# relife957/FastApriori

Measured on AMD Instinct MI355X. Metric: itemsets/sec (mining wall-clock), T10I4D100M min_sup=0.001, higher is better.
Workload: dtype int32/uint64-bitmap (exact integer counts); 1 GPU; model=T10I4D100M, global_batch=100000000, parallelism=dp1, n_itemsets=33139, min_count=100000

## Files before the change

### csrc/hip/fa_hip.h

```cpp
#pragma once
#include <hip/hip_runtime.h>
#include <stdint.h>

#define FA_API extern "C" __attribute__((visibility("default")))

#define FA_LAUNCH_RET() return (int)hipGetLastError()

namespace fa {

constexpr int kWave = 64;

__device__ __forceinline__ int lane_id() { return (int)(threadIdx.x & 63); }

__device__ __forceinline__ uint32_t popc64_acc(uint64_t x, uint32_t acc) {
  return acc + (uint32_t)__popc((uint32_t)x) + (uint32_t)__popc((uint32_t)(x >> 32));
}

__device__ __forceinline__ int wave_scan_incl_dpp(int v) {
  const int lane = (int)(threadIdx.x & 63);
  const int r = lane & 15;
  int t;
  t = __builtin_amdgcn_update_dpp(0, v, 0x111, 0xf, 0xf, false); if (r >= 1) v += t;
  t = __builtin_amdgcn_update_dpp(0, v, 0x112, 0xf, 0xf, false); if (r >= 2) v += t;
  t = __builtin_amdgcn_update_dpp(0, v, 0x114, 0xf, 0xf, false); if (r >= 4) v += t;
// ... 157 lines not shown
  for (int i = 0, j = 0; i < k - 1; ++i, ++j) {
    if (j == p) ++j;
    const int32_t x = a[i], y = s[j];
    if (x != y) return x < y ? -1 : 1;
  }
  return 0;
}

struct DlDesc;

}

FA_API int fa_hip_dl_plan(const fa::DlDesc* desc, int L, long long* ctl, int F1, int32_t* item_map, void* rec,
                          int64_t max_pieces, int32_t* part, int64_t part_cap, int32_t* gpre, int64_t gpre_cap,
                          int sw, hipStream_t st);
FA_API int fa_hip_count_slab_rec_cls(const int64_t* roff, const int32_t* ranks, const int32_t* src, int64_t ncols,
                                     const int32_t* item_map, int F1, int n_used, const int32_t* gpre,
                                     const void* rec, int G, int C, const int32_t* wword, uint32_t* out, int sw,
                                     int n_wg, const uint64_t* bm, int64_t Wp, hipStream_t st,
                                     const int32_t* bm_rows, const int32_t* g_dev, int cls);
```

### csrc/hip/gen.hip

```cpp
#include <hipcub/hipcub.hpp>

#include <algorithm>
#include <cmath>

#include "fa_hip.h"
#include "../host/fa_dl.h"
#include "../host/fa_limits.h"
#include "../host/fa_slab.h"

namespace fa {

__device__ __forceinline__ uint64_t ag_mix(uint64_t x) {
  x ^= x >> 33; x *= 0xff51afd7ed558ccdull; x ^= x >> 33; x *= 0xc4ceb9fe1a85ec53ull; x ^= x >> 33;
  return x;
}

__device__ __forceinline__ uint64_t ag_hash_drop(const int32_t* __restrict__ r, int m, int skip) {
  uint64_t h = 0x9E3779B97F4A7C15ull ^ (uint64_t)(m - 1);
  for (int q = 0; q < m; ++q)
    if (q != skip) h = ag_mix(h ^ (uint32_t)r[q]);
  return h;
}

__device__ __forceinline__ bool ag_eq_drop(const int32_t* __restrict__ a, const int32_t* __restrict__ b, int m,
// ... 845 lines not shown
  int64_t Cl[kDlMaxL], C = 0, R = 0;
  for (int l = 0; l < *L; ++l) { Cl[l] = desc[l].C; C += desc[l].C; R += desc[l].n; }
  const int64_t n_used = ch[kDlNUsed];
  const int Lp = *Lp_out = slab_tail_cut(Cl, *L, n_used, lds, accb_rule);
  if (Lp == *L) return false;
  const bool ends = ch[kDlEmpty] || (g_tail_levels > 0 && *L == g_tail_levels);
  if (ends && C <= P->rec_cap && C <= P->out_cap && 8 * ((R + 255) / 256) <= P->part_cap &&
      slab_pack_width(n_used, C, lds, accb_pack, cap, pad) == 16 && C <= *cap) {
    *sw = 16;
    return true;
  }
  dl_tail_cut(desc, L, Lp, ch);
  return false;
}

static void dl_post(DlPost* P, const DlDesc* desc, int L, long long* ctl, long long* ch, int F1,
                    double accb_rule, double accb_pack, double lds, hipStream_t st) {
  P->done = 0;
  if (ch[kDlStop] && ch[kDlLevels] == 0) return;
  if (ch[kDlOverBound] || ch[kDlMulti] || ch[kDlEnd] || L < 1) return;
  int64_t cap = 0;
  int sw = 0, pad = 0, Lp = L;
  const bool packed = accb_pack > 0.0 && dl_tail(P, desc, &L, ch, accb_rule, accb_pack, lds, &Lp, &sw, &cap, &pad);
  int64_t C = 0, R = 0;
  for (int l = 0; l < L; ++l) { C += desc[l].C; R += desc[l].n; }
  const int64_t n_used = ch[kDlNUsed];
  P->C = C;
  if (C < 1 || C > P->rec_cap || C > P->out_cap || 8 * ((R + 255) / 256) > P->part_cap) return;
  double accb = accb_rule;
  if (packed) {
    accb = accb_pack;
  } else {
    sw = slab_width(n_used, C, P->lds_budget, accb_rule, &cap);
    if (sw == 0 || C > cap) return;
    if (!P->wword) slab_acc_upgrade(n_used, C, P->lds_budget, P->accb, &sw, &cap, &accb);
  }
  P->accb = accb;
  if (fa_hip_dl_plan(desc, L, ctl, F1, P->item_map, P->rec, C, P->part, P->part_cap, P->gpre, P->gpre_cap,
                     slab_layout(sw, pad), st) != 0) {
    if (packed) dl_tail_cut(desc, &L, Lp, ch);
    return;
  }
  (void)hipMemsetAsync(P->out, 0, 4 * (size_t)C, st);
  P->sw = slab_layout(sw, pad);
  P->cap = cap;
  P->done = 1;
  P->trim = 0;
  if (!P->trim_ok || P->T <= 0) {
  } else if (!P->len_hist || P->T < P->trim_min_rows) {
    if (!P->len_hist && P->T >= P->trim_min_rows) return;
  } else {
    const uint64_t* mk = reinterpret_cast<const uint64_t*>(ch + kDlBits);
    double num = 0.0, den = 0.0;
    for (int r = 0; r < F1; ++r) {
      if (P->alive[r]) den += (double)P->c1[r];
      if ((mk[r >> 6] >> (r & 63)) & 1ull) num += (double)P->c1[r];
    }
    if (den > 0.0) {
      double est_rows = 0.0, est_nnz = 0.0;
      trim_estimate(P->len_hist, kTrimHist, num / den, (int)P->k, &est_rows, &est_nnz);
      const double T = (double)std::max<int64_t>(P->T, 1), nnz = (double)std::max<int64_t>(P->nnz, 1);
      P->trim = (est_rows < P->trim_rows_frac * T || est_nnz < P->trim_nnz_frac * nnz) ? 1 : 0;
    }
  }
  if (P->trim) return;
  const int64_t W = (P->ncols + 63) / 64, nslabs = (W + sw - 1) / sw;
  const bool weighted = P->wword != nullptr;
  const int64_t nacc = slab_acc_count(C, slab_acc_bytes(P->accb, weighted));
  P->n_wg = slab_workgroups(nslabs, (int64_t)P->lds_kernel,
                            slab_kernel_lds_pack(n_used, sw, pad, slab_acc_words(nacc), slab_map_lds(F1)));
  if (fa_hip_count_slab_rec_cls(P->roff, P->ranks, P->src, P->ncols, P->item_map, F1, (int)n_used, P->gpre, P->rec,
                                0, (int)C, P->wword, P->out, slab_layout(sw, pad), (int)P->n_wg, nullptr, 0, st,
                                nullptr,
                                reinterpret_cast<const int32_t*>(ctl + kDlPiecesI32),
                                slab_acc_mode(P->accb, weighted)) != 0)
    return;
  P->done = 2;
}

FA_API int fa_hip_dl_more(int F1, void* ws, int64_t ws_bytes, int64_t ws_used, long long* ctl, long long* ctl_host,
                          double growth, int max_levels, double lds, double accb, int64_t n1_bound, fa::DlDesc* desc,
                          int64_t* info, hipStream_t st, void* post) {
  using namespace fa;
  auto al = [](int64_t b) { return (b + 255) & ~(int64_t)255; };
  const int nw = (F1 + 63) / 64;
  char* const w0 = static_cast<char*>(ws);
  char* w = w0 + ws_used;
  const int LM = std::min(max_levels, kDlMaxLevels);
  const int64_t acc_max = (int64_t)(lds / accb);
  const DlPost* const tp = static_cast<const DlPost*>(post);
  const double accb_pack = tp && !tp->wword && F1 <= kSlabMapMaxF1 ? g_tail_accb : 0.0;
  int64_t nb = n1_bound;
// ... 87 lines not shown
  desc[0].C = ctl_host[kDlCl];
  desc[0].base = 0;
  const int L = (int)ctl_host[kDlLevels];
  for (int l = 1; l < L; ++l) {
    DlDesc& d = desc[l];
    d.P = desc[l - 1].rows;
    d.cnt = (int64_t)(intptr_t)lv[l].cnt;
    d.off = (int64_t)(intptr_t)lv[l].off;
    d.rows = (int64_t)(intptr_t)lv[l].rows;
    d.m = lv[l].m;
    d.n = ctl_host[kDlNl + l];
    d.C = ctl_host[kDlCl + l];
    d.base = desc[l - 1].base + desc[l - 1].C;
  }
  info[0] = w - w0;
  if (post) dl_post(static_cast<DlPost*>(post), desc, L, ctl, ctl_host, F1, accb, accb_pack, lds, st);
  FA_LAUNCH_RET();
}
```

### fastapriori_amd/models/apriori.py

```python
from __future__ import annotations

import gc
import math
import os
import time
from dataclasses import dataclass

import numpy as np
import torch

from .. import ops
from ..ops.host import apriori_gen
from ..parallel.comm import Comm
from ..tuning import TUNING
from ..utils.jvm import item_tiebreak_key, min_count
from ..utils.metrics import Logger, Timer, roctx_range
from .data import MiningResult, TransactionShard

HORIZONTAL_PAIRS_PER_S = 2.0e11
GRAM_WORDPAIRS_PER_S = 1.7e13
F1_SKETCH_MIN_VOCAB = 1 << 20
F1_HIST_READBACK = 1 << 16
_TRIU_CACHE: dict = {}
_POW10 = 10 ** np.arange(1, 11, dtype=np.int64)
# ... 269 lines not shown
        S = Pm.device_level_state(self._dev)
        F1 = self._F1
        lds = Pm.dl_lds_budget(F1)
        unit = db["wword"] is None
        self._dl_mp_accb = 2.0 if TUNING.dl_acc16 and unit else 4.0
        acc8 = int(TUNING.dl_acc8_bundles) if unit else 0
        if int(self._count_view(db)["ncols"]) < TUNING.dl_acc8_min_rows:
            acc8 = 0
        accb = self._dl_accb = 1.0 if acc8 == 1 else 2.0 if TUNING.dl_acc16_bundles and unit else 4.0
        self._dl_cnt_accb = 1.0 if acc8 == 2 else accb
        counters = 1 if self.cand_par else max(1, self.comm.world_size)
        tail_rows = int(self.stats["n_lines"]) // counters
        self._dl_tail_accb = 0.0
        if TUNING.dl_tail_bundle and unit and Pm.slab_map_lds(F1) > 0 and tail_rows >= TUNING.dl_acc8_min_rows:
            self._dl_tail_accb = 1.0 if int(TUNING.dl_acc8_bundles) else 2.0 if TUNING.dl_acc16_bundles else 4.0
        c_bound = int(lds // accb)
        st = torch.cuda.current_stream(self._dev).cuda_stream
        f2 = self._f2_dev
        m0, k = 2, 3
        if f2 is None:
            last = np.ascontiguousarray(levels[-1], dtype=np.int32)
            m0, k = last.shape[1], last.shape[1] + 1
            f2 = self._resume_rows = torch.from_numpy(last.reshape(-1, m0)).to(self._dev)
        if self._f2_n_dev is not None:
            P0, n_src, n_const, n_bound = f2.data_ptr(), self._f2_n_dev.data_ptr(), 0, self._f2_bound
        else:
            P0, n_src, n_const, n_bound = f2.data_ptr(), None, int(f2.shape[0]), int(f2.shape[0])
        if self.ckpt is not None and self._ckpt_deferred:
            self._result_items(result)
            n_host = next((i for i, lv in enumerate(levels) if lv is None), len(levels))
# ... 15 lines not shown
                tail_levels = 0
                if self.cfg.max_level and self.cfg.max_level - k + 1 <= max_lv:
                    max_lv = tail_levels = self.cfg.max_level - k + 1
                if not TUNING.bundle_levels or k - 1 > TUNING.bundle_max_prefix:
                    max_lv = 1
                post = TUNING.dl_post and max_lv > 1
                S.rows_hint = int(self._count_view(db)["ncols"])
                if post:
                    self._dl_post_setup(S, db, k, F1, c_bound, n_bound, lds)
                if pend:
                    self._dl_stage(S, pend)
                with roctx_range("gen"):
                    c = Pm.dl_bundle_gen(S, P0, n_src, n_const, n_bound, m0, F1, c_bound, lds, TUNING.bundle_growth,
                                         max_lv, st, post=post, accb=accb,
                                         tail_accb=self._dl_tail_accb if post else 0.0,
                                         tail_levels=tail_levels if max_lv > 1 else 0)
                if c[K.kDlOverBound]:
                    raise RuntimeError(f"device bundle at level {k}: |F_{k - 1}| exceeds its bound {n_bound}")
                if c[K.kDlEnd]:
                    break
                multi = None
                if c[K.kDlMulti]:
                    multi = self._dl_multipass(S, db, k, F1, c, P0, n_src, n_const, n_bound, m0, lds, st)
                    if multi is None:
                        nxt = k
                        break
                    c = multi[0]
                L, n_used = int(c[K.kDlLevels]), int(c[K.kDlNUsed])
                Cs = S.desc["C"][:L].copy()
                C = int(Cs.sum())
                done = int(S.post.done) if post else 0
# ... 985 lines not shown
```

### fastapriori_amd/ops/_native.py

```python
from __future__ import annotations

import ctypes as C
import os
import threading

from . import build as _build

_lock = threading.Lock()
_host = None
_hip = None

i32, i64, u64, dbl = C.c_int32, C.c_int64, C.c_uint64, C.c_double
vp, cp = C.c_void_p, C.c_char_p
I64P = C.POINTER(C.c_int64)
IP = C.POINTER(C.c_int)

_HOST_SIGS = {
    "fa_parse_file": (vp, [cp, i64, i64, C.c_int, C.c_int, IP]),
    "fa_parse_buffer": (vp, [cp, i64, C.c_int, C.c_int]),
    "fa_file_size": (i64, [cp]),
    "fa_next_line_start": (i64, [cp, i64, i64]),
    "fa_chunk_scan": (None, [vp, i64, vp]),
    "fa_txndb_info": (None, [vp, vp]),
    "fa_txndb_export": (None, [vp, vp, vp, vp, C.c_int]),
    "fa_txndb_export_dict": (None, [vp, vp, vp, vp, C.c_int]),
    "fa_hash_tokens": (None, [vp, vp, i64, vp, C.c_int]),
    "fa_txndb_free": (None, [vp]),
    "fa_hash_bytes": (u64, [cp, i64]),
    "fa_quest_generate": (vp, [i64, i64, dbl, dbl, i64, i64, u64, C.c_int, C.c_int]),
    "fa_zipf_generate": (vp, [i64, i64, dbl, dbl, i64, dbl, dbl, i64, u64, C.c_int]),
    "fa_zipf_write": (C.c_int, [cp, i64, dbl, dbl, i64, dbl, dbl, i64, u64, C.c_int, C.c_int]),
    "fa_quest_write": (C.c_int, [cp, i64, dbl, dbl, i64, i64, u64, C.c_int, C.c_int]),
    "fa_apriori_gen": (vp, [vp, i64, C.c_int, C.c_int, vp]),
    "fa_cands_export": (None, [vp, vp, vp, vp]),
    "fa_cands_free": (None, [vp]),
    "fa_level_plan": (C.c_int, [vp, vp, i64, vp, vp, i32, vp, vp, i64, vp, i64, vp]),
    "fa_slab_width": (C.c_int, [i64, i64, dbl, dbl, I64P]),
    "fa_slab_total_limit": (i64, [i64, dbl, dbl]),
    "fa_slab_map_lds": (i64, [i64]),
    "fa_slab_workgroups": (i64, [i64, i64, C.c_int, i64, C.c_int, i64, i64]),
    "fa_slab_acc_mode": (C.c_int, [dbl, C.c_int, i64, I64P]),
    "fa_slab_acc_upgrade": (C.c_int, [i64, i64, dbl, dbl, C.POINTER(C.c_int), I64P, C.POINTER(dbl)]),
    "fa_slab_row_off": (i64, [C.c_int, C.c_int, i64]),
    "fa_slab_row_col": (C.c_int, [C.c_int, C.c_int, i64]),
    "fa_slab_rows_bytes": (i64, [C.c_int, C.c_int, i64]),
    "fa_slab_layout": (C.c_int, [C.c_int, C.c_int]),
    "fa_slab_pack_width": (C.c_int, [i64, i64, dbl, dbl, I64P, C.POINTER(C.c_int)]),
    "fa_slab_tail_cut": (C.c_int, [vp, C.c_int, i64, dbl, dbl]),
    "fa_trim_estimate": (None, [vp, i64, dbl, C.c_int, C.POINTER(dbl), C.POINTER(dbl)]),
    "fa_dl_layout": (cp, [C.c_int, I64P]),
    "fa_limits": (cp, [C.c_int, I64P]),
# ... 56 lines not shown
    "fa_hip_lr_rows": (C.c_int, [vp, vp, vp, i64, vp, C.c_int, vp, i64, vp]),
    "fa_hip_compress_regs_bc": (C.c_int, [vp, vp, vp, vp, i64, vp, vp, vp, vp, vp, i64, C.c_int, vp]),
    "fa_hip_block_counts_rows": (C.c_int, [vp, vp, vp, i64, vp, i64, C.c_int, vp, vp]),
    "fa_hip_block_bsum": (C.c_int, [vp, i64, i64, C.c_int, vp, vp]),
    "fa_hip_compress_staged": (C.c_int, [vp, vp, vp, i64, vp, vp, vp, vp, vp]),
    "fa_hip_compress_staged64": (C.c_int, [vp, vp, vp, i64, vp, vp, vp, vp, C.c_int, vp]),
    "fa_hip_count_slab_rec_cls": (C.c_int, [vp, vp, vp, i64, vp, C.c_int, C.c_int, vp, vp, C.c_int, C.c_int, vp,
                                            vp, C.c_int, C.c_int, vp, i64, vp, vp, vp, C.c_int]),
    "fa_hip_dl_level0": (C.c_int, [vp, vp, i64, i64, C.c_int, C.c_int, vp, i64, vp, vp, i64, dbl, dbl, vp, C.c_int,
                                   vp]),
    "fa_hip_dl_more": (C.c_int, [C.c_int, vp, i64, i64, vp, vp, dbl, C.c_int, dbl, dbl, i64, vp, vp, vp, vp]),
    "fa_hip_dl_plan": (C.c_int, [vp, C.c_int, vp, C.c_int, vp, vp, i64, vp, i64, vp, i64, C.c_int, vp]),
    "fa_hip_set_lane_deal": (None, [C.c_int]),
    "fa_hip_set_dl_tail": (None, [dbl, C.c_int]),
    "fa_hip_set_piece_part": (C.c_int, [C.c_int, C.c_int]),
    "fa_hip_dl_gpre_need": (i64, [vp, C.c_int]),
    "fa_hip_dl_plan_window": (C.c_int, [vp, C.c_int, vp, C.c_int, vp, vp, i64, vp, i64, vp, i64, i64, i64, C.c_int,
                                        vp]),
    "fa_hip_dl_plan_window_bits": (C.c_int, [vp, C.c_int, vp, C.c_int, vp, vp, vp, i64, vp, i64, vp, i64, i64, i64,
                                             C.c_int, vp]),
    "fa_hip_dl_chunk_bits": (C.c_int, [vp, C.c_int, C.c_int, vp, vp]),
    "fa_hip_dl_threshold": (C.c_int, [vp, C.c_int, vp, i64, vp, vp, vp, vp, vp, vp, i64, vp]),
    "fa_hip_trim_scan_count": (C.c_int, [vp, vp, i64, vp, C.c_int, C.c_int, vp, vp, vp, vp, vp]),
    "fa_hip_trim_emit": (C.c_int, [vp, vp, vp, C.c_int, i64, vp, vp, vp, vp, vp, vp, vp, vp]),
    "fa_hip_compress_wave": (C.c_int, [vp, vp, vp, vp, i64, vp, vp, vp, C.c_int, vp, vp]),
    "fa_hip_compress_lds": (C.c_int, [vp, vp, vp, vp, i64, vp, vp, vp, vp, vp, vp]),
    "fa_hip_dedup_probe": (C.c_int, [vp, vp, vp, i64, vp, vp, vp]),
    "fa_hip_row_hash": (C.c_int, [vp, vp, i64, vp, vp, vp]),
    "fa_hip_build_bitmaps": (C.c_int, [vp, vp, vp, i64, i32, i64, C.c_int, C.c_int, vp, vp, vp, C.c_int, vp]),
    "fa_hip_block_counts": (C.c_int, [vp, vp, i64, i32, vp, vp, C.c_int, vp]),
# ... 97 lines not shown
```

### fastapriori_amd/ops/build.py

```python
from __future__ import annotations

import glob
import hashlib
import os
import shutil
import subprocess
import sys

HERE = os.path.dirname(os.path.abspath(__file__))
ROOT = os.path.dirname(os.path.dirname(HERE))
CSRC = os.path.join(ROOT, "csrc")
HOST_LIB = os.path.join(HERE, "libfa_host.so")
HIP_LIB = os.path.join(HERE, "libfa_hip.so")
ARCH = os.environ.get("PYTORCH_ROCM_ARCH", "gfx950").split(";")[0] or "gfx950"

HOST_FLAGS = ["-O3", "-std=c++17", "-shared", "-fPIC", "-pthread", "-mpopcnt", "-fvisibility=hidden", "-Wall",
              "-Wno-unused-function"]
ASAN_FLAGS = ["-O1", "-g", "-std=c++17", "-shared", "-fPIC", "-pthread", "-mpopcnt",
              "-fsanitize=address,undefined", "-fno-omit-frame-pointer"]
HIP_FLAGS = [f"--offload-arch={ARCH}", "-O3", "-std=c++17", "-shared", "-fPIC", "-fvisibility=hidden",
             "-Wno-unused-result"]
_MARKER = b"FA_BUILD_ID:"


# ... 10 lines not shown
        raise RuntimeError(f"build failed: {' '.join(cmd)}\n{r.stdout}\n{r.stderr}")


def host_sources() -> list[str]:
    return sorted(glob.glob(os.path.join(CSRC, "host", "*.cpp")))


def hip_sources() -> list[str]:
    return sorted(glob.glob(os.path.join(CSRC, "hip", "*.hip")))


def _deps(kind: str) -> list[str]:
    if kind == "host":
        return host_sources() + sorted(glob.glob(os.path.join(CSRC, "host", "*.h")))
    return hip_sources() + sorted(glob.glob(os.path.join(CSRC, "hip", "*.h"))) + [
        os.path.join(CSRC, "host", h) for h in ("fa_dl.h", "fa_limits.h", "fa_query.h", "fa_rule_measures.h",
                                                "fa_slab.h")]


def source_id(kind: str, flags: list[str] | None = None) -> str:
    if flags is None:
        flags = HOST_FLAGS if kind == "host" else HIP_FLAGS
    h = hashlib.sha256()
    for p in _deps(kind):
        h.update(os.path.relpath(p, ROOT).encode() + b"\0")
        with open(p, "rb") as f:
            h.update(f.read())
        h.update(b"\0")
    h.update(" ".join(flags).encode())
    return h.hexdigest()[:16]


# ... 43 lines not shown
```

### fastapriori_amd/ops/host.py

```python
from __future__ import annotations

import ctypes as C
from dataclasses import dataclass, field

import numpy as np

from ..config import RULE_SORTS
from ..utils.env import num_threads
from . import _native


def apriori_gen(prev: np.ndarray):
    prev = np.ascontiguousarray(prev, dtype=np.int32)
    n, m = prev.shape
    sizes = np.zeros(2, dtype=np.int64)
    lib = _native.host()
    h = lib.fa_apriori_gen(prev.ctypes.data, n, m, num_threads(), sizes.ctypes.data)
    G, Cn = int(sizes[0]), int(sizes[1])
    prefix = np.zeros(max(G, 1), dtype=np.int32)
    ext_off = np.zeros(G + 1, dtype=np.int64)
    ext = np.zeros(max(Cn, 1), dtype=np.int32)
    lib.fa_cands_export(h, prefix.ctypes.data, ext_off.ctypes.data, ext.ctypes.data)
    lib.fa_cands_free(h)
    return prefix[:G], ext_off, ext[:Cn]


@dataclass
class RuleTable:
    ante_off: np.ndarray
    ante: np.ndarray
    cons: np.ndarray
    conf: np.ndarray
    level_stats: list
    level_ms: list = field(default_factory=list)

    @property
    def n_rules(self) -> int:
        return int(self.cons.size)

# ... 141 lines not shown
```

### fastapriori_amd/ops/primitives.py

```python
from __future__ import annotations

import ctypes as C
import ctypes
import functools
import os
import time
from dataclasses import dataclass

import numpy as np
import torch

from ..tuning import TUNING
from ..utils.env import num_threads
from . import _native
from .host import rule_measures_plan, rules_gap_level, rules_not_closed

_I32, _I64 = torch.int32, torch.int64
PAIR_CHUNK_ROWS = 1 << 18


def _p(t: torch.Tensor | None) -> int | None:
    return None if t is None else t.data_ptr()


# ... 1683 lines not shown
def device_level_state(dev) -> DeviceLevelState:
    st = _DL_STATE.get(dev)
    if st is None:
        st = _DL_STATE[dev] = DeviceLevelState(dev)
    return st


def dl_lds_budget(F1: int) -> int:
    return TUNING.slab_lds_bytes - slab_map_lds(F1)




def dl_bundle_gen(S: DeviceLevelState, P0: int, n_src: int | None, n_const: int, n_bound: int, m0: int, F1: int,
                  c_bound: int, lds: int, growth: float, max_levels: int, stream: int, post: bool = False,
                  accb: float = 4.0, tail_accb: float = 0.0, tail_levels: int = 0) -> np.ndarray:
    lib, K = _native.hip(), dl()
    info = np.zeros(2, dtype=np.int64)
    for _ in range(6):
        S.desc[:] = 0
        rc = lib.fa_hip_dl_level0(P0, n_src, n_const, n_bound, m0, F1, _p(S.ws), S.ws.numel(), _p(S.ctl),
                                  _p(S.ctl_h), c_bound, float(lds), float(accb), S.info.ctypes.data,
                                  int(max_levels <= 1), stream)
        if rc == 5:
            S.grow(int(S.info[0]))
            continue
        _native.check(rc, "fa_hip_dl_level0")
        d0 = S.desc[0]
        d0["P"], d0["cnt"], d0["off"], d0["rows"], d0["m"] = P0, S.info[1], S.info[2], S.info[3], m0
        if max_levels <= 1:
            c = S.ctl_h.numpy()
            d0["n"], d0["C"], d0["base"] = c[K.kDlNl], c[K.kDlCl], 0
            return c.copy()
        S.post.done = 0
        lane_deal(lib, S.rows_hint)
        lib.fa_hip_set_dl_tail(float(tail_accb) if post else 0.0, int(tail_levels))
        rc = lib.fa_hip_dl_more(F1, _p(S.ws), S.ws.numel(), int(S.info[0]), _p(S.ctl), _p(S.ctl_h), float(growth),
                                int(max_levels), float(lds), float(accb), int(c_bound), S.desc.ctypes.data,
                                info.ctypes.data,
                                stream, ctypes.addressof(S.post) if post else None)
        if rc == 5:
            S.grow(int(info[0]))
            continue
        _native.check(rc, "fa_hip_dl_more")
        return S.ctl_h.numpy().copy()
    raise RuntimeError("device bundle generation: workspace sizing did not converge")


def set_piece_part(part: int, nparts: int) -> None:
    _native.check(_native.hip().fa_hip_set_piece_part(int(part), int(nparts)), "fa_hip_set_piece_part")


def lane_deal(lib, rows: int) -> None:
    lib.fa_hip_set_lane_deal(int(0 <= TUNING.lane_deal_min_rows <= rows))


def dl_plan(S: DeviceLevelState, L: int, F1: int, n_used: int, C: int, lds: int, dev, accb: float = 4.0,
            cnt_accb: float | None = None, pad: int = 0) -> dict:
    st = torch.cuda.current_stream(dev).cuda_stream
    sw, cap = slab_width(n_used, C, lds, accb)
    if sw == 0 or C > cap:
        raise RuntimeError(f"device bundle of {C} candidates over {n_used} items does not fit one pass")
    if cnt_accb is not None and cnt_accb < accb:
        sw_c, cap_c, accb_c = ctypes.c_int(sw), ctypes.c_int64(cap), ctypes.c_double(accb)
        _native.host().fa_slab_acc_upgrade(int(n_used), int(C), float(lds), float(cnt_accb), ctypes.byref(sw_c),
                                           ctypes.byref(cap_c), ctypes.byref(accb_c))
        sw, cap, accb = int(sw_c.value), int(cap_c.value), float(accb_c.value)
    item_map = torch.empty(max(F1, 1), dtype=_I32, device=dev)
    rec = torch.empty(12 * C + 12, dtype=_I32, device=dev)
    R = int(S.desc["n"][:L].sum())
    part = torch.empty(8 * max(1, (R + 255) // 256), dtype=_I32, device=dev)
    lib = _native.hip()
    gn = int(lib.fa_hip_dl_gpre_need(S.desc.ctypes.data, L))
    gpre = torch.empty(max(gn, 1), dtype=_I32, device=dev)
    lane_deal(lib, S.rows_hint)
    _native.check(lib.fa_hip_dl_plan(S.desc.ctypes.data, L, _p(S.ctl), F1, _p(item_map), _p(rec), C,
                                     _p(part), part.numel(), _p(gpre), gpre.numel(), slab_layout(sw, pad), st),
                  "fa_hip_dl_plan")
    out = torch.zeros(C, dtype=_I32, device=dev)
    return dict(sw=sw, pad=pad, cap=cap, item_map=item_map, rec=rec, out=out, n_used=n_used, C=C, gpre=gpre,
                accb=accb)


def dl_count_multipass(S: DeviceLevelState, F1: int, n_used: int, C: int, lds: int, roff, ranks, src, ncols: int,
                       wword, bm, bm_rows, sup_frac: float, dev, bmap=None, window_rows=None) -> torch.Tensor | None:
    acc16 = TUNING.dl_acc16 and wword is None
    accb = 2 if acc16 else 4
    sw, cap = slab_width(n_used, C, lds, accb)
    if sw == 0:
        return None
    st = _stream(ranks)
# ... 164 lines not shown
```

### fastapriori_amd/tuning.py

```python
from __future__ import annotations

import os
from contextlib import contextmanager
from dataclasses import dataclass, fields


@dataclass
class Tuning:
    bundle_levels: bool = True
    bundle_growth: float = 1.5
    bundle_max_prefix: int = 9
    device_levels: bool = True
    dl_post: bool = True
    dl_multi: bool = True
    gen_device: bool = True
    gen_chain: bool = True
    gen_device_min_rows: int = 512
    pair_rs_min: int = 1 << 22
    fused_compress: bool = True
    early_compress: bool = True
    f1_rank_device: bool = True
    fused_compress_mean_len: float = 12.0
    fused_layout: bool = True
    compress_wave_mean_len: float = 48.0
    slab_lds_bytes: int = 160 * 1024 - 512
    slab_cls: int = 1
    dense_min_rows: float = 4.0
    dl_acc16: bool = True
    dl_acc16_bundles: bool = False
    dl_acc8_bundles: int = 2
    dl_acc8_min_rows: int = 1 << 20
    dl_tail_bundle: bool = True
    mp_window_items: bool = True
    window_trim: bool = True
    window_trim_est_frac: float = 0.95
    window_trim_rows_frac: float = 0.97
    window_trim_cost: float = 100.0
    window_trim_min_rows: int = 1 << 25
    lane_deal_min_rows: int = 1 << 25
    pair_wg: int = 0
    gram_mfma_min_class_words: int = 512
    bitmap_blocked: bool = True
    trim_rows_frac: float = 0.75
    trim_nnz_frac: float = 0.6
    query_lds_bytes: int = 160 * 1024 - 512
    query_acc: int = 0
    query_max_wg: int = 0
# ... 47 lines not shown
```

Measured before the change: 903,300 itemsets/s.

## Regroup bundled candidates under shared parent prefixes before slab counting

Adds a GPU regroup kernel that reassigns each candidate to one of its (k-1)-subset parents, greedily favouring parents with many candidates. The goal is fewer prefix pieces in the slab counting plan, so there is less intersection work per piece. Counts land in a permuted buffer and an unpermute kernel restores the original order. The kernel keeps the original grouping when it is no better. The cost is an extra regroup launch, scratch workspace (possibly forcing a workspace regrow), an extra memset and an unpermute pass.

```diff
diff --git a/csrc/hip/fa_hip.h b/csrc/hip/fa_hip.h
--- a/csrc/hip/fa_hip.h
+++ b/csrc/hip/fa_hip.h
@@ -195,6 +195,10 @@
 FA_API int fa_hip_dl_plan(const fa::DlDesc* desc, int L, long long* ctl, int F1, int32_t* item_map, void* rec,
                           int64_t max_pieces, int32_t* part, int64_t part_cap, int32_t* gpre, int64_t gpre_cap,
                           int sw, hipStream_t st);
+FA_API int64_t fa_hip_dl_regroup_need(const fa::DlDesc* desc, int L);
+FA_API int fa_hip_dl_regroup(const fa::DlDesc* desc, int L, void* scratch, int64_t bytes, fa::DlDesc* out,
+                             long long* stats, hipStream_t st);
+FA_API int fa_hip_dl_unpermute(const uint32_t* in, const int32_t* perm, int64_t C, uint32_t* out, hipStream_t st);
 FA_API int fa_hip_count_slab_rec_cls(const int64_t* roff, const int32_t* ranks, const int32_t* src, int64_t ncols,
                                      const int32_t* item_map, int F1, int n_used, const int32_t* gpre,
                                      const void* rec, int G, int C, const int32_t* wword, uint32_t* out, int sw,
diff --git a/csrc/hip/gen.hip b/csrc/hip/gen.hip
--- a/csrc/hip/gen.hip
+++ b/csrc/hip/gen.hip
@@ -6,6 +6,7 @@
 #include "fa_hip.h"
 #include "../host/fa_dl.h"
 #include "../host/fa_limits.h"
+#include "../host/fa_regroup.h"
 #include "../host/fa_slab.h"
 
 namespace fa {
@@ -883,11 +884,32 @@
   return false;
 }
 
-static void dl_post(DlPost* P, const DlDesc* desc, int L, long long* ctl, long long* ch, int F1,
-                    double accb_rule, double accb_pack, double lds, hipStream_t st) {
+static int g_regroup = 0;
+FA_API void fa_hip_set_dl_regroup(int on) { g_regroup = on; }
+static int64_t g_regroup_last[2] = {0, 0};
+FA_API void fa_hip_dl_regroup_last(int64_t* out) {
+  for (int i = 0; i < 2; ++i) out[i] = g_regroup_last[i];
+}
+
+static int64_t dl_regroup_ws(const DlDesc* desc, int L) {
+  if (!g_regroup) return 0;
+  const int64_t need = fa_hip_dl_regroup_need(desc, L);
+  if (need == 0) return 0;
+  int64_t C = 0;
+  for (int l = 0; l < L; ++l) C += desc[l].C;
+  return need + ((4 * C + 255) & ~(int64_t)255);
+}
+
+static bool dl_post_skips(const long long* ch, int L) {
+  if (ch[kDlStop] && ch[kDlLevels] == 0) return true;
+  return ch[kDlOverBound] || ch[kDlMulti] || ch[kDlEnd] || L < 1;
+}
+
+static int64_t dl_post(DlPost* P, const DlDesc* desc, int L, long long* ctl, long long* ch, int F1,
+                    double accb_rule, double accb_pack, double lds, char* free_ws, int64_t free_bytes,
+                    hipStream_t st) {
   P->done = 0;
-  if (ch[kDlStop] && ch[kDlLevels] == 0) return;
-  if (ch[kDlOverBound] || ch[kDlMulti] || ch[kDlEnd] || L < 1) return;
+  if (dl_post_skips(ch, L)) return 0;
   int64_t cap = 0;
   int sw = 0, pad = 0, Lp = L;
   const bool packed = accb_pack > 0.0 && dl_tail(P, desc, &L, ch, accb_rule, accb_pack, lds, &Lp, &sw, &cap, &pad);
@@ -895,29 +917,21 @@
   for (int l = 0; l < L; ++l) { C += desc[l].C; R += desc[l].n; }
   const int64_t n_used = ch[kDlNUsed];
   P->C = C;
-  if (C < 1 || C > P->rec_cap || C > P->out_cap || 8 * ((R + 255) / 256) > P->part_cap) return;
+  if (C < 1 || C > P->rec_cap || C > P->out_cap || 8 * ((R + 255) / 256) > P->part_cap) return 0;
   double accb = accb_rule;
   if (packed) {
     accb = accb_pack;
   } else {
     sw = slab_width(n_used, C, P->lds_budget, accb_rule, &cap);
-    if (sw == 0 || C > cap) return;
+    if (sw == 0 || C > cap) return 0;
     if (!P->wword) slab_acc_upgrade(n_used, C, P->lds_budget, P->accb, &sw, &cap, &accb);
   }
   P->accb = accb;
-  if (fa_hip_dl_plan(desc, L, ctl, F1, P->item_map, P->rec, C, P->part, P->part_cap, P->gpre, P->gpre_cap,
-                     slab_layout(sw, pad), st) != 0) {
-    if (packed) dl_tail_cut(desc, &L, Lp, ch);
-    return;
-  }
-  (void)hipMemsetAsync(P->out, 0, 4 * (size_t)C, st);
-  P->sw = slab_layout(sw, pad);
-  P->cap = cap;
-  P->done = 1;
-  P->trim = 0;
+  int trim = 0;
+  bool caller_decides = false;
   if (!P->trim_ok || P->T <= 0) {
   } else if (!P->len_hist || P->T < P->trim_min_rows) {
-    if (!P->len_hist && P->T >= P->trim_min_rows) return;
+    caller_decides = !P->len_hist && P->T >= P->trim_min_rows;
   } else {
     const uint64_t* mk = reinterpret_cast<const uint64_t*>(ch + kDlBits);
     double num = 0.0, den = 0.0;
@@ -929,22 +943,53 @@
       double est_rows = 0.0, est_nnz = 0.0;
       trim_estimate(P->len_hist, kTrimHist, num / den, (int)P->k, &est_rows, &est_nnz);
       const double T = (double)std::max<int64_t>(P->T, 1), nnz = (double)std::max<int64_t>(P->nnz, 1);
-      P->trim = (est_rows < P->trim_rows_frac * T || est_nnz < P->trim_nnz_frac * nnz) ? 1 : 0;
-    }
-  }
-  if (P->trim) return;
+      trim = (est_rows < P->trim_rows_frac * T || est_nnz < P->trim_nnz_frac * nnz) ? 1 : 0;
+    }
+  }
+  DlDesc rg[kDlMaxL];
+  const DlDesc* pd = desc;
+  const int32_t* perm = nullptr;
+  uint32_t* cnt_rg = nullptr;
+  const int64_t rg_bytes = (trim || caller_decides) ? 0 : dl_regroup_ws(desc, L);
+  if (rg_bytes > free_bytes) return rg_bytes;
+  if (rg_bytes > 0) {
+    const int64_t cb = (4 * C + 255) & ~(int64_t)255;
+    if (fa_hip_dl_regroup(desc, L, free_ws + cb, free_bytes - cb, rg, ctl + kRgStats, st) == 0) {
+      pd = rg;
+      perm = reinterpret_cast<const int32_t*>(free_ws + cb);
+      cnt_rg = reinterpret_cast<uint32_t*>(free_ws);
+      ++g_regroup_last[0];
+      g_regroup_last[1] = L;
+    }
+  }
+  if (fa_hip_dl_plan(pd, L, ctl, F1, P->item_map, P->rec, C, P->part, P->part_cap, P->gpre, P->gpre_cap,
+                     slab_layout(sw, pad), st) != 0) {
+    if (packed) dl_tail_cut(desc, &L, Lp, ch);
+    return 0;
+  }
+  (void)hipMemsetAsync(P->out, 0, 4 * (size_t)C, st);
+  if (cnt_rg) (void)hipMemsetAsync(cnt_rg, 0, 4 * (size_t)C, st);
+  P->sw = slab_layout(sw, pad);
+  P->cap = cap;
+  P->done = 1;
+  P->trim = trim;
+  if (caller_decides || trim) return 0;
   const int64_t W = (P->ncols + 63) / 64, nslabs = (W + sw - 1) / sw;
   const bool weighted = P->wword != nullptr;
   const int64_t nacc = slab_acc_count(C, slab_acc_bytes(P->accb, weighted));
   P->n_wg = slab_workgroups(nslabs, (int64_t)P->lds_kernel,
                             slab_kernel_lds_pack(n_used, sw, pad, slab_acc_words(nacc), slab_map_lds(F1)));
   if (fa_hip_count_slab_rec_cls(P->roff, P->ranks, P->src, P->ncols, P->item_map, F1, (int)n_used, P->gpre, P->rec,
-                                0, (int)C, P->wword, P->out, slab_layout(sw, pad), (int)P->n_wg, nullptr, 0, st,
-                                nullptr,
+                                0, (int)C, P->wword, cnt_rg ? cnt_rg : P->out, slab_layout(sw, pad), (int)P->n_wg,
+                                nullptr, 0, st, nullptr,
                                 reinterpret_cast<const int32_t*>(ctl + kDlPiecesI32),
-                                slab_acc_mode(P->accb, weighted)) != 0)
-    return;
+                                slab_acc_mode(P->accb, weighted)) != 0 ||
+      (cnt_rg && fa_hip_dl_unpermute(cnt_rg, perm, C, P->out, st) != 0)) {
+    if (cnt_rg) P->done = 0;
+    return 0;
+  }
   P->done = 2;
+  return 0;
 }
 
 FA_API int fa_hip_dl_more(int F1, void* ws, int64_t ws_bytes, int64_t ws_used, long long* ctl, long long* ctl_host,
@@ -1062,6 +1107,13 @@
     d.base = desc[l - 1].base + desc[l - 1].C;
   }
   info[0] = w - w0;
-  if (post) dl_post(static_cast<DlPost*>(post), desc, L, ctl, ctl_host, F1, accb, accb_pack, lds, st);
+  if (post) {
+    const int64_t more = dl_post(static_cast<DlPost*>(post), desc, L, ctl, ctl_host, F1, accb, accb_pack, lds, w,
+                                 ws_bytes - (w - w0), st);
+    if (more > 0) {
+      info[0] = 2 * ((w - w0) + more);
+      return 5;
+    }
+  }
   FA_LAUNCH_RET();
 }
diff --git a/csrc/hip/regroup.hip b/csrc/hip/regroup.hip
--- /dev/null
+++ b/csrc/hip/regroup.hip
@@ -0,0 +1,255 @@
+#include "fa_hip.h"
+#include "../host/fa_dl.h"
+#include "../host/fa_regroup.h"
+
+namespace fa {
+
+constexpr int kRgThreads = 1024;
+constexpr int kRgW = kRgThreads / 64;
+
+struct RgLv {
+  const int32_t* P;
+  const int32_t* cnt;
+  const int64_t* off;
+  const int32_t* rows;
+  char* scr;
+  int64_t n, C, base;
+  int64_t m;
+};
+struct RgArgs {
+  RgLv lv[kDlMaxL];
+  int32_t* perm;
+  long long* stats;
+};
+
+__host__ __device__ inline int64_t rg_scratch_ints(int64_t n, int64_t C, int64_t m) {
+  return ((C * (m + 5) + n) + 1) & ~(int64_t)1;
+}
+__host__ __device__ inline int64_t rg_scratch_bytes(int64_t n, int64_t C, int64_t m) {
+  return (4 * rg_scratch_ints(n, C, m) + 8 * (n + 1) + 255) & ~(int64_t)255;
+}
+
+__device__ __forceinline__ int rg_find(const int32_t* __restrict__ P, int n, int m, const int32_t* __restrict__ s,
+                                       int j) {
+  int lo = 0, hi = n;
+  while (lo < hi) {
+    const int mid = (lo + hi) >> 1;
+    const int r = cmp_skip(P + (int64_t)mid * m, s, m + 1, j);
+    if (r == 0) return mid;
+    if (r < 0) lo = mid + 1; else hi = mid;
+  }
+  return -1;
+}
+
+__global__ __launch_bounds__(kRgThreads) void k_dl_regroup(const RgArgs A) {
+  extern __shared__ int rg_lds[];
+  __shared__ int sh[2 * kRgW];
+  __shared__ int fired;
+  const RgLv& V = A.lv[blockIdx.x];
+  const int tid = threadIdx.x;
+  const int64_t C = V.C, base = V.base;
+  if (V.n > kRgMaxRows) {
+    for (int64_t c = tid; c < C; c += kRgThreads) A.perm[base + c] = (int32_t)(base + c);
+    int pp = 0;
+    for (int64_t i = tid; i < V.n; i += kRgThreads) pp += (V.cnt[i] + 7) >> 3;
+    pp = wg_sum<kRgW>(pp, sh);
+    if (tid == 0) {
+      long long* s = A.stats + 4 * blockIdx.x;
+      s[0] = s[1] = pp; s[2] = 0; s[3] = 1;
+    }
+    return;
+  }
+  const int n = (int)V.n, m = (int)V.m, k = m + 1;
+  int32_t* const par = reinterpret_cast<int32_t*>(V.scr);
+  int32_t* const asg = par + C * k;
+  int32_t* const cho = asg + C;
+  int32_t* const tmp = cho + C;
+  int32_t* const cnt_out = tmp + C;
+  int32_t* const ex_out = cnt_out + n;
+  int64_t* const off_out = reinterpret_cast<int64_t*>(V.scr + 4 * rg_scratch_ints(n, C, m));
+  int* u = rg_lds;
+  int* u2 = rg_lds + n;
+  int* const v = rg_lds + 2 * n;
+  for (int i = tid; i < 3 * n; i += kRgThreads) rg_lds[i] = 0;
+  if (tid == 0) fired = 0;
+  __syncthreads();
+  for (int64_t c = tid; c < C; c += kRgThreads) {
+    const int32_t* s = V.rows + c * k;
+    int lo = 0, hi = n;
+    while (lo < hi) {
+      const int mid = (lo + hi) >> 1;
+      if (V.off[mid] <= c) lo = mid + 1; else hi = mid;
+    }
+    for (int j = 0; j < m; ++j) par[c * k + j] = rg_find(V.P, n, m, s, j);
+    par[c * k + m] = lo - 1;
+    asg[c] = -1;
+    for (int j = 0; j < k; ++j) {
+      const int p = par[c * k + j];
+      if (p >= 0) atomicAdd(&u[p], 1);
+    }
+  }
+  __syncthreads();
+  int rounds = 0;
+  for (int t = 0; t < kRgNThr; ++t) {
+    const int thr = rg_thr(t);
+    for (;;) {
+      ++rounds;
+      for (int64_t c = tid; c < C; c += kRgThreads) {
+        if (asg[c] >= 0) continue;
+        int best = -1, bp = -1;
+        for (int j = k - 1; j >= 0; --j) {
+          const int p = par[c * k + j];
+          if (p < 0) continue;
+          const int uu = u[p];
+          if (uu >= thr && uu > best) { best = uu; bp = p; }
+        }
+        cho[c] = bp;
+        if (bp >= 0) atomicAdd(&v[bp], 1);
+      }
+      __syncthreads();
+      for (int64_t c = tid; c < C; c += kRgThreads) {
+        if (asg[c] >= 0) continue;
+        const int bp = cho[c];
+        if (bp >= 0 && v[bp] >= thr) {
+          asg[c] = bp;
+          fired = 1;
+          continue;
+        }
+        for (int j = 0; j < k; ++j) {
+          const int p = par[c * k + j];
+          if (p >= 0) atomicAdd(&u2[p], 1);
+        }
+      }
+      __syncthreads();
+      const int f = fired;
+      __syncthreads();
+      if (tid == 0) fired = 0;
+      if (f) { int* x = u; u = u2; u2 = x; }
+      for (int i = tid; i < n; i += kRgThreads) { u2[i] = 0; v[i] = 0; }
+      __syncthreads();
+      if (!f) break;
+    }
+  }
+  for (int64_t c = tid; c < C; c += kRgThreads) atomicAdd(&v[asg[c]], 1);
+  __syncthreads();
+  int pc[2] = {0, 0}, tot[2];
+  for (int i = tid; i < n; i += kRgThreads) {
+    pc[0] += (v[i] + 7) >> 3;
+    pc[1] += (V.cnt[i] + 7) >> 3;
+  }
+  wg_sum<kRgW>(pc, sh, tot);
+  const bool keep = tot[0] >= tot[1];
+  __syncthreads();
+  if (keep) {
+    for (int i = tid; i < n; i += kRgThreads) v[i] = 0;
+    __syncthreads();
+    for (int64_t c = tid; c < C; c += kRgThreads) {
+      asg[c] = par[c * k + m];
+      atomicAdd(&v[asg[c]], 1);
+    }
+    __syncthreads();
+  }
+  for (int i = tid; i < n; i += kRgThreads) cnt_out[i] = v[i];
+  wg_scan_chunks<kRgW>(
+      (int64_t)n, (int64_t)0, sh, [&](int64_t i) { return v[i]; },
+      [&](int64_t i, int64_t before, int) { off_out[i] = before; });
+  if (tid == 0) off_out[n] = C;
+  for (int64_t c = tid; c < C; c += kRgThreads) {
+    const int p = asg[c];
+    tmp[off_out[p] + atomicAdd(&u2[p], 1)] = (int32_t)c;
+  }
+  __syncthreads();
+  for (int64_t c = tid; c < C; c += kRgThreads) {
+    const int p = asg[c];
+    const int64_t o = off_out[p];
+    const int a = v[p];
+    int r = 0;
+    for (int q = 0; q < a; ++q) r += tmp[o + q] < (int32_t)c ? 1 : 0;
+    int j = m;
+    if (!keep)
+      for (j = k - 1; j > 0 && par[c * k + j] != p; --j) {}
+    ex_out[o + r] = V.rows[c * k + j];
+    A.perm[base + o + r] = (int32_t)(base + c);
+  }
+  if (tid == 0) {
+    long long* s = A.stats + 4 * blockIdx.x;
+    s[0] = tot[1]; s[1] = tot[0]; s[2] = rounds; s[3] = keep ? 1 : 0;
+  }
+}
+
+__global__ __launch_bounds__(256) void k_dl_unpermute(const uint32_t* __restrict__ in, const int32_t* __restrict__ perm,
+                                                      int64_t C, uint32_t* __restrict__ out) {
+  const int64_t e = (int64_t)blockIdx.x * 256 + threadIdx.x;
+  if (e < C) out[perm[e]] = in[e];
+}
+
+static inline int64_t rg_al(int64_t b) { return (b + 255) & ~(int64_t)255; }
+
+static bool rg_eligible(const DlDesc* desc, int L) {
+  if (L < 1 || L > kDlMaxL) return false;
+  for (int l = 0; l < L; ++l)
+    if (desc[l].m < 1 || desc[l].m > kDlInline || desc[l].n < 1 || desc[l].C < 1 || desc[l].C > INT32_MAX / 64)
+      return false;
+  return true;
+}
+
+}
+
+using namespace fa;
+
+FA_API int64_t fa_hip_dl_regroup_need(const DlDesc* desc, int L) {
+  if (!rg_eligible(desc, L)) return 0;
+  int64_t C = 0, b = 0;
+  for (int l = 0; l < L; ++l) {
+    C += desc[l].C;
+    if (desc[l].n <= kRgMaxRows) b += rg_scratch_bytes(desc[l].n, desc[l].C, desc[l].m);
+  }
+  return rg_al(4 * C) + b;
+}
+
+FA_API int fa_hip_dl_regroup(const DlDesc* desc, int L, void* scratch, int64_t bytes, DlDesc* out, long long* stats,
+                             hipStream_t st) {
+  const int64_t need = fa_hip_dl_regroup_need(desc, L);
+  if (need == 0 || scratch == nullptr || stats == nullptr || bytes < need) return 1;
+  int64_t C = 0;
+  for (int l = 0; l < L; ++l) C += desc[l].C;
+  RgArgs A{};
+  char* w = static_cast<char*>(scratch);
+  A.perm = reinterpret_cast<int32_t*>(w);
+  w += rg_al(4 * C);
+  A.stats = stats;
+  int64_t n_max = 1;
+  for (int l = 0; l < L; ++l) {
+    const DlDesc& d = desc[l];
+    RgLv& V = A.lv[l];
+    V.P = reinterpret_cast<const int32_t*>((intptr_t)d.P);
+    V.cnt = reinterpret_cast<const int32_t*>((intptr_t)d.cnt);
+    V.off = reinterpret_cast<const int64_t*>((intptr_t)d.off);
+    V.rows = reinterpret_cast<const int32_t*>((intptr_t)d.rows);
+    V.n = d.n; V.C = d.C; V.base = d.base; V.m = d.m;
+    V.scr = w;
+    out[l] = d;
+    if (d.n > kRgMaxRows) continue;
+    n_max = std::max(n_max, d.n);
+    int32_t* cnt_out = reinterpret_cast<int32_t*>(w) + d.C * (d.m + 1) + 3 * d.C;
+    out[l].cnt = (int64_t)(intptr_t)cnt_out;
+    out[l].off = (int64_t)(intptr_t)(w + 4 * rg_scratch_ints(d.n, d.C, d.m));
+    w += rg_scratch_bytes(d.n, d.C, d.m);
+  }
+  const size_t lds = 3 * sizeof(int) * (size_t)n_max;
+  static bool lds_set = false;
+  if (!lds_set) {
+    const hipError_t e = hipFuncSetAttribute((const void*)k_dl_regroup, hipFuncAttributeMaxDynamicSharedMemorySize,
+                                             (int)(3 * sizeof(int) * kRgMaxRows));
+    if (e != hipSuccess) return (int)e;
+    lds_set = true;
+  }
+  hipLaunchKernelGGL(k_dl_regroup, dim3((unsigned)L), dim3(kRgThreads), lds, st, A);
+  FA_LAUNCH_RET();
+}
+
+FA_API int fa_hip_dl_unpermute(const uint32_t* in, const int32_t* perm, int64_t C, uint32_t* out, hipStream_t st) {
+  if (C < 1) return 1;
+  hipLaunchKernelGGL(k_dl_unpermute, dim3((unsigned)((C + 255) / 256)), dim3(256), 0, st, in, perm, C, out);
+  FA_LAUNCH_RET();
+}
diff --git a/csrc/host/fa_regroup.h b/csrc/host/fa_regroup.h
--- /dev/null
+++ b/csrc/host/fa_regroup.h
@@ -0,0 +1,21 @@
+#pragma once
+#include <stdint.h>
+
+namespace fa {
+
+constexpr int kRgNThr = 6;
+constexpr int rg_thr(int t) { return t == 0 ? 8 : t == 1 ? 6 : t == 2 ? 4 : t == 3 ? 3 : t == 4 ? 2 : 1; }
+constexpr int kRgMaxRows = 12288;
+constexpr int kRgStats = 224;
+static_assert(kRgStats + 4 * 32 <= 512, "the statistics end before the control block's bitset");
+
+inline int rg_cmp_skip(const int32_t* a, const int32_t* s, int k, int p) {
+  for (int i = 0, j = 0; i < k - 1; ++i, ++j) {
+    if (j == p) ++j;
+    const int32_t x = a[i], y = s[j];
+    if (x != y) return x < y ? -1 : 1;
+  }
+  return 0;
+}
+
+}
diff --git a/csrc/host/regroup.cpp b/csrc/host/regroup.cpp
--- /dev/null
+++ b/csrc/host/regroup.cpp
@@ -0,0 +1,121 @@
+#include <algorithm>
+#include <vector>
+
+#include "fa_common.h"
+#include "fa_dl.h"
+#include "fa_regroup.h"
+
+namespace fa {
+
+struct RgLevel {
+  const int32_t* P;
+  const int32_t* cnt;
+  const int64_t* off;
+  const int32_t* ex;
+  int64_t n, C, m;
+  int32_t* cnt_out;
+  int64_t* off_out;
+  int32_t* ex_out;
+  int32_t* perm;
+  int64_t pieces_prefix, pieces_rule, rounds, kept_prefix;
+};
+static_assert(sizeof(RgLevel) == 15 * 8, "RgLevel layout (ops.host.RgLevelC)");
+
+static int64_t rg_find(const int32_t* P, int64_t n, int m, const int32_t* s, int j) {
+  int64_t lo = 0, hi = n;
+  while (lo < hi) {
+    const int64_t mid = (lo + hi) >> 1;
+    const int r = rg_cmp_skip(P + mid * m, s, m + 1, j);
+    if (r == 0) return mid;
+    if (r < 0) lo = mid + 1; else hi = mid;
+  }
+  return -1;
+}
+
+static int64_t rg_pieces(const std::vector<int32_t>& a) {
+  int64_t p = 0;
+  for (int32_t c : a) p += (c + 7) / 8;
+  return p;
+}
+
+static void rg_level(RgLevel& lv, bool regroup) {
+  const int64_t n = lv.n, C = lv.C;
+  const int m = (int)lv.m, k = m + 1;
+  std::vector<int64_t> pre(C), asg(C, -1), par;
+  for (int64_t i = 0; i < n; ++i)
+    for (int64_t c = lv.off[i]; c < lv.off[i] + lv.cnt[i]; ++c) pre[c] = i;
+  std::vector<int32_t> a_pre(lv.cnt, lv.cnt + n);
+  lv.pieces_prefix = lv.pieces_rule = rg_pieces(a_pre);
+  lv.rounds = 0;
+  lv.kept_prefix = 1;
+  if (regroup && n <= kRgMaxRows) {
+    par.assign(C * k, -1);
+    std::vector<int32_t> row(k);
+    for (int64_t c = 0; c < C; ++c) {
+      std::copy(lv.P + pre[c] * m, lv.P + pre[c] * m + m, row.begin());
+      row[m] = lv.ex[c];
+      for (int j = 0; j < m; ++j) par[c * k + j] = rg_find(lv.P, n, m, row.data(), j);
+      par[c * k + m] = pre[c];
+    }
+    std::vector<int32_t> u(n), v(n);
+    std::vector<int64_t> cho(C);
+    for (int t = 0; t < kRgNThr; ++t) {
+      const int thr = rg_thr(t);
+      for (;;) {
+        ++lv.rounds;
+        std::fill(u.begin(), u.end(), 0);
+        std::fill(v.begin(), v.end(), 0);
+        for (int64_t c = 0; c < C; ++c)
+          if (asg[c] < 0)
+            for (int j = 0; j < k; ++j)
+              if (par[c * k + j] >= 0) ++u[par[c * k + j]];
+        for (int64_t c = 0; c < C; ++c) {
+          if (asg[c] >= 0) continue;
+          int best = -1;
+          int64_t bp = -1;
+          for (int j = k - 1; j >= 0; --j) {
+            const int64_t p = par[c * k + j];
+            if (p >= 0 && u[p] >= thr && u[p] > best) { best = u[p]; bp = p; }
+          }
+          cho[c] = bp;
+          if (bp >= 0) ++v[bp];
+        }
+        bool fired = false;
+        for (int64_t c = 0; c < C; ++c)
+          if (asg[c] < 0 && cho[c] >= 0 && v[cho[c]] >= thr) { asg[c] = cho[c]; fired = true; }
+        if (!fired) break;
+      }
+    }
+    std::vector<int32_t> a(n, 0);
+    for (int64_t c = 0; c < C; ++c) ++a[asg[c]];
+    lv.pieces_rule = rg_pieces(a);
+    lv.kept_prefix = lv.pieces_rule < lv.pieces_prefix ? 0 : 1;
+  }
+  if (lv.kept_prefix) asg = pre;
+  std::fill(lv.cnt_out, lv.cnt_out + n, 0);
+  for (int64_t c = 0; c < C; ++c) ++lv.cnt_out[asg[c]];
+  lv.off_out[0] = 0;
+  for (int64_t i = 0; i < n; ++i) lv.off_out[i + 1] = lv.off_out[i] + lv.cnt_out[i];
+  std::vector<int64_t> cur(lv.off_out, lv.off_out + n);
+  for (int64_t c = 0; c < C; ++c) {
+    const int64_t p = asg[c], at = cur[p]++;
+    int j = m;
+    if (!lv.kept_prefix)
+      for (j = k - 1; j > 0 && par[c * k + j] != p; --j) {}
+    lv.ex_out[at] = j == m ? lv.ex[c] : lv.P[pre[c] * m + j];
+    lv.perm[at] = (int32_t)c;
+  }
+}
+
+}
+
+using namespace fa;
+
+FA_API int fa_dl_regroup(RgLevel* lv, int L) {
+  bool ok = true;
+  for (int l = 0; l < L; ++l) ok = ok && lv[l].m <= kDlInline;
+  for (int l = 0; l < L; ++l) rg_level(lv[l], ok);
+  return ok ? 1 : 0;
+}
+
+FA_API int64_t fa_dl_regroup_const(int i) { return i == 0 ? kRgMaxRows : i == 1 ? kRgStats : -1; }
diff --git a/fastapriori_amd/models/apriori.py b/fastapriori_amd/models/apriori.py
--- a/fastapriori_amd/models/apriori.py
+++ b/fastapriori_amd/models/apriori.py
@@ -307,6 +307,7 @@
         self._dl_tail_accb = 0.0
         if TUNING.dl_tail_bundle and unit and Pm.slab_map_lds(F1) > 0 and tail_rows >= TUNING.dl_acc8_min_rows:
             self._dl_tail_accb = 1.0 if int(TUNING.dl_acc8_bundles) else 2.0 if TUNING.dl_acc16_bundles else 4.0
+        regroup = bool(TUNING.dl_regroup) and tail_rows >= TUNING.dl_regroup_min_rows
         c_bound = int(lds // accb)
         st = torch.cuda.current_stream(self._dev).cuda_stream
         f2 = self._f2_dev
@@ -352,7 +353,7 @@
                     c = Pm.dl_bundle_gen(S, P0, n_src, n_const, n_bound, m0, F1, c_bound, lds, TUNING.bundle_growth,
                                          max_lv, st, post=post, accb=accb,
                                          tail_accb=self._dl_tail_accb if post else 0.0,
-                                         tail_levels=tail_levels if max_lv > 1 else 0)
+                                         tail_levels=tail_levels if max_lv > 1 else 0, regroup=regroup)
                 if c[K.kDlOverBound]:
                     raise RuntimeError(f"device bundle at level {k}: |F_{k - 1}| exceeds its bound {n_bound}")
                 if c[K.kDlEnd]:
diff --git a/fastapriori_amd/ops/_native.py b/fastapriori_amd/ops/_native.py
--- a/fastapriori_amd/ops/_native.py
+++ b/fastapriori_amd/ops/_native.py
@@ -35,6 +35,8 @@
     "fa_cands_export": (None, [vp, vp, vp, vp]),
     "fa_cands_free": (None, [vp]),
     "fa_level_plan": (C.c_int, [vp, vp, i64, vp, vp, i32, vp, vp, i64, vp, i64, vp]),
+    "fa_dl_regroup": (C.c_int, [vp, C.c_int]),
+    "fa_dl_regroup_const": (i64, [C.c_int]),
     "fa_slab_width": (C.c_int, [i64, i64, dbl, dbl, I64P]),
     "fa_slab_total_limit": (i64, [i64, dbl, dbl]),
     "fa_slab_map_lds": (i64, [i64]),
@@ -121,6 +123,11 @@
     "fa_hip_set_lane_deal": (None, [C.c_int]),
     "fa_hip_set_dl_tail": (None, [dbl, C.c_int]),
     "fa_hip_set_piece_part": (C.c_int, [C.c_int, C.c_int]),
+    "fa_hip_set_dl_regroup": (None, [C.c_int]),
+    "fa_hip_dl_regroup_last": (None, [vp]),
+    "fa_hip_dl_regroup_need": (i64, [vp, C.c_int]),
+    "fa_hip_dl_regroup": (C.c_int, [vp, C.c_int, vp, i64, vp, vp, vp]),
+    "fa_hip_dl_unpermute": (C.c_int, [vp, vp, i64, vp, vp]),
     "fa_hip_dl_gpre_need": (i64, [vp, C.c_int]),
     "fa_hip_dl_plan_window": (C.c_int, [vp, C.c_int, vp, C.c_int, vp, vp, i64, vp, i64, vp, i64, i64, i64, C.c_int,
                                         vp]),
diff --git a/fastapriori_amd/ops/build.py b/fastapriori_amd/ops/build.py
--- a/fastapriori_amd/ops/build.py
+++ b/fastapriori_amd/ops/build.py
@@ -48,8 +48,8 @@
     if kind == "host":
         return host_sources() + sorted(glob.glob(os.path.join(CSRC, "host", "*.h")))
     return hip_sources() + sorted(glob.glob(os.path.join(CSRC, "hip", "*.h"))) + [
-        os.path.join(CSRC, "host", h) for h in ("fa_dl.h", "fa_limits.h", "fa_query.h", "fa_rule_measures.h",
-                                                "fa_slab.h")]
+        os.path.join(CSRC, "host", h) for h in ("fa_dl.h", "fa_limits.h", "fa_query.h", "fa_regroup.h",
+                                                "fa_rule_measures.h", "fa_slab.h")]
 
 
 def source_id(kind: str, flags: list[str] | None = None) -> str:
diff --git a/fastapriori_amd/ops/host.py b/fastapriori_amd/ops/host.py
--- a/fastapriori_amd/ops/host.py
+++ b/fastapriori_amd/ops/host.py
@@ -23,6 +23,42 @@
     lib.fa_cands_export(h, prefix.ctypes.data, ext_off.ctypes.data, ext.ctypes.data)
     lib.fa_cands_free(h)
     return prefix[:G], ext_off, ext[:Cn]
+
+
+class RgLevelC(C.Structure):
+    _fields_ = [(n, C.c_void_p) for n in ("P", "cnt", "off", "ex")] + \
+               [(n, C.c_int64) for n in ("n", "C", "m")] + \
+               [(n, C.c_void_p) for n in ("cnt_out", "off_out", "ex_out", "perm")] + \
+               [(n, C.c_int64) for n in ("pieces_prefix", "pieces_rule", "rounds", "kept_prefix")]
+
+
+def dl_regroup(levels) -> tuple[bool, list[dict]]:
+    L = len(levels)
+    arr = (RgLevelC * L)()
+    keep, out = [], []
+    for l, (P, cnt, ex) in enumerate(levels):
+        P = np.ascontiguousarray(P, dtype=np.int32)
+        cnt = np.ascontiguousarray(cnt, dtype=np.int32)
+        ex = np.ascontiguousarray(ex, dtype=np.int32)
+        n, m = P.shape
+        Cn = int(ex.size)
+        assert cnt.shape == (n,) and int(cnt.sum()) == Cn
+        off = np.concatenate([[0], np.cumsum(cnt, dtype=np.int64)]).astype(np.int64)
+        o = dict(cnt=np.zeros(n, np.int32), off=np.zeros(n + 1, np.int64), ex=np.zeros(max(Cn, 1), np.int32),
+                 perm=np.zeros(max(Cn, 1), np.int32))
+        keep.append((P, cnt, ex, off))
+        a = arr[l]
+        a.P, a.cnt, a.off, a.ex = P.ctypes.data, cnt.ctypes.data, off.ctypes.data, ex.ctypes.data
+        a.n, a.C, a.m = n, Cn, m
+        a.cnt_out, a.off_out, a.ex_out, a.perm = (o[k].ctypes.data for k in ("cnt", "off", "ex", "perm"))
+        out.append(o)
+    regrouped = bool(_native.host().fa_dl_regroup(C.addressof(arr), L))
+    for l, o in enumerate(out):
+        Cn = int(arr[l].C)
+        o["ex"], o["perm"] = o["ex"][:Cn], o["perm"][:Cn]
+        for k in ("pieces_prefix", "pieces_rule", "rounds", "kept_prefix"):
+            o[k] = int(getattr(arr[l], k))
+    return regrouped, out
 
 
 @dataclass
diff --git a/fastapriori_amd/ops/primitives.py b/fastapriori_amd/ops/primitives.py
--- a/fastapriori_amd/ops/primitives.py
+++ b/fastapriori_amd/ops/primitives.py
@@ -1721,7 +1721,8 @@
 
 def dl_bundle_gen(S: DeviceLevelState, P0: int, n_src: int | None, n_const: int, n_bound: int, m0: int, F1: int,
                   c_bound: int, lds: int, growth: float, max_levels: int, stream: int, post: bool = False,
-                  accb: float = 4.0, tail_accb: float = 0.0, tail_levels: int = 0) -> np.ndarray:
+                  accb: float = 4.0, tail_accb: float = 0.0, tail_levels: int = 0,
+                  regroup: bool | None = None) -> np.ndarray:
     lib, K = _native.hip(), dl()
     info = np.zeros(2, dtype=np.int64)
     for _ in range(6):
@@ -1742,6 +1743,7 @@
         S.post.done = 0
         lane_deal(lib, S.rows_hint)
         lib.fa_hip_set_dl_tail(float(tail_accb) if post else 0.0, int(tail_levels))
+        lib.fa_hip_set_dl_regroup(int(bool(TUNING.dl_regroup if regroup is None else regroup) and post))
         rc = lib.fa_hip_dl_more(F1, _p(S.ws), S.ws.numel(), int(S.info[0]), _p(S.ctl), _p(S.ctl_h), float(growth),
                                 int(max_levels), float(lds), float(accb), int(c_bound), S.desc.ctypes.data,
                                 info.ctypes.data,
@@ -1762,8 +1764,42 @@
     lib.fa_hip_set_lane_deal(int(0 <= TUNING.lane_deal_min_rows <= rows))
 
 
+def dl_regroup(S: DeviceLevelState, L: int, dev) -> dict | None:
+    lib = _native.hip()
+    need = int(lib.fa_hip_dl_regroup_need(S.desc.ctypes.data, L))
+    if need == 0:
+        return None
+    scratch = torch.empty(need, dtype=torch.uint8, device=dev)
+    stats = torch.zeros((L, 4), dtype=_I64, device=dev)
+    desc = S.desc.copy()
+    st = torch.cuda.current_stream(dev).cuda_stream
+    _native.check(lib.fa_hip_dl_regroup(S.desc.ctypes.data, L, _p(scratch), need, desc.ctypes.data, _p(stats), st),
+                  "fa_hip_dl_regroup")
+    C = int(S.desc["C"][:L].sum())
+    perm = scratch[:4 * C].view(_I32)
+    return dict(desc=desc, perm=perm, stats=stats, scratch=scratch)
+
+
+def dl_regroup_last(S: DeviceLevelState | None = None) -> tuple[int, np.ndarray | None]:
+    last = np.zeros(2, dtype=np.int64)
+    _native.hip().fa_hip_dl_regroup_last(last.ctypes.data)
+    S = S if S is not None else next(iter(_DL_STATE.values()), None)
+    if last[0] == 0 or S is None:
+        return int(last[0]), None
+    at, L = int(_native.host().fa_dl_regroup_const(1)), int(last[1])
+    return int(last[0]), S.ctl[at:at + 4 * L].cpu().numpy().reshape(L, 4)
+
+
+def dl_unpermute(cnt: torch.Tensor, perm: torch.Tensor) -> torch.Tensor:
+    out = torch.empty_like(cnt)
+    st = torch.cuda.current_stream(cnt.device).cuda_stream
+    _native.check(_native.hip().fa_hip_dl_unpermute(_p(cnt), _p(perm), cnt.numel(), _p(out), st),
+                  "fa_hip_dl_unpermute")
+    return out
+
+
 def dl_plan(S: DeviceLevelState, L: int, F1: int, n_used: int, C: int, lds: int, dev, accb: float = 4.0,
-            cnt_accb: float | None = None, pad: int = 0) -> dict:
+            cnt_accb: float | None = None, pad: int = 0, desc=None) -> dict:
     st = torch.cuda.current_stream(dev).cuda_stream
     sw, cap = slab_width(n_used, C, lds, accb)
     if sw == 0 or C > cap:
@@ -1775,13 +1811,14 @@
         sw, cap, accb = int(sw_c.value), int(cap_c.value), float(accb_c.value)
     item_map = torch.empty(max(F1, 1), dtype=_I32, device=dev)
     rec = torch.empty(12 * C + 12, dtype=_I32, device=dev)
-    R = int(S.desc["n"][:L].sum())
+    desc = S.desc if desc is None else desc
+    R = int(desc["n"][:L].sum())
     part = torch.empty(8 * max(1, (R + 255) // 256), dtype=_I32, device=dev)
     lib = _native.hip()
-    gn = int(lib.fa_hip_dl_gpre_need(S.desc.ctypes.data, L))
+    gn = int(lib.fa_hip_dl_gpre_need(desc.ctypes.data, L))
     gpre = torch.empty(max(gn, 1), dtype=_I32, device=dev)
     lane_deal(lib, S.rows_hint)
-    _native.check(lib.fa_hip_dl_plan(S.desc.ctypes.data, L, _p(S.ctl), F1, _p(item_map), _p(rec), C,
+    _native.check(lib.fa_hip_dl_plan(desc.ctypes.data, L, _p(S.ctl), F1, _p(item_map), _p(rec), C,
                                      _p(part), part.numel(), _p(gpre), gpre.numel(), slab_layout(sw, pad), st),
                   "fa_hip_dl_plan")
     out = torch.zeros(C, dtype=_I32, device=dev)
diff --git a/fastapriori_amd/tuning.py b/fastapriori_amd/tuning.py
--- a/fastapriori_amd/tuning.py
+++ b/fastapriori_amd/tuning.py
@@ -31,6 +31,8 @@
     dl_acc8_bundles: int = 2
     dl_acc8_min_rows: int = 1 << 20
     dl_tail_bundle: bool = True
+    dl_regroup: bool = True
+    dl_regroup_min_rows: int = 1 << 26
     mp_window_items: bool = True
     window_trim: bool = True
     window_trim_est_frac: float = 0.95
```

New measurement: 921,600 itemsets/s, median of 6. +2.0%, better.
